# prashantpandeygit/solvingpapers

Measured on AMD Instinct MI355X. Metric: training tokens/sec, LLaMA3-8B-shape bf16, higher is better.
Workload: dtype bf16; 1 GPU; model=llama3_8b, global_batch=4, seq_len=8192, parallelism=dp1, micro_batch=1, grad_accum=4, params=8030261248

## Files before the change

### csrc/include/attn_common.h

```cpp
#pragma once
#include "spa_common.h"
#include <type_traits>

namespace spa {

template <int HD> constexpr int img_w() { return HD == 192 ? 256 : HD; }

typedef short s16x4 __attribute__((ext_vector_type(4)));
typedef int i32x4 __attribute__((ext_vector_type(4)));

constexpr float kRescaleThr = 8.f;

__device__ __forceinline__ f32x16 mfma32(const bf16x8& a, const bf16x8& b, const f32x16& c) {
  return __builtin_amdgcn_mfma_f32_32x32x16_bf16(a, b, c, 0, 0, 0);
}
__device__ __forceinline__ float fexp2(float x) { return __builtin_amdgcn_exp2f(x); }
__device__ __forceinline__ float halfmax(float x) {
  const auto r = __builtin_amdgcn_permlane32_swap(__float_as_uint(x), __float_as_uint(x), false, false);
  return fmaxf(__uint_as_float(r[0]), __uint_as_float(r[1]));
}
__device__ __forceinline__ float halfsum(float x) {
  const auto r = __builtin_amdgcn_permlane32_swap(__float_as_uint(x), __float_as_uint(x), false, false);
  return __uint_as_float(r[0]) + __uint_as_float(r[1]);
}
// ... 60 lines not shown
    for (int dt = 0; dt < NTR; ++dt) {
      const int c = 32 * dt + 16 * (g & 1) + 4 * pp;
      const int ch = c >> 3, within = c & 7;
      tra.v[dt] = ra * HD + 8 * (ch ^ swz<HD>(ra)) + within;
      trb.v[dt] = rb * HD + 8 * (ch ^ swz<HD>(rb)) + within;
    }
    SPA_DBG_LDS(row.v[NR - 1] + 7, 32 * HD);
    SPA_DBG_LDS(trb.v[NTR - 1] + 3, 16 * HD);
  }
};
__device__ __forceinline__ bf16x8 ld_row(const bf16* img, int off) {
  return *reinterpret_cast<const bf16x8*>(img + off);
}
__device__ __forceinline__ bf16x8 ld_tr(const bf16* img, int offa, int offb) {
  typedef __attribute__((address_space(3))) s16x4 lds_s4;
  const s16x4 a = __builtin_amdgcn_ds_read_tr16_b64_v4i16((lds_s4*)(img + offa));
  const s16x4 b = __builtin_amdgcn_ds_read_tr16_b64_v4i16((lds_s4*)(img + offb));
  const bf16x4 av = __builtin_bit_cast(bf16x4, a), bv = __builtin_bit_cast(bf16x4, b);
  return __builtin_shufflevector(av, bv, 0, 1, 2, 3, 4, 5, 6, 7);
}
template <int V> using IC = std::integral_constant<int, V>;

template <int N, int PER, int AHEAD, int PRE = 0>
__device__ __forceinline__ void chain_sched() {
  __builtin_amdgcn_sched_group_barrier(0x100, PRE + AHEAD * PER, 0);
#pragma unroll
  for (int i = 0; i < N - AHEAD; ++i) {
    __builtin_amdgcn_sched_group_barrier(0x008, 1, 0);
    __builtin_amdgcn_sched_group_barrier(0x100, PER, 0);
  }
  __builtin_amdgcn_sched_group_barrier(0x008, AHEAD, 0);
}

__device__ __forceinline__ unsigned lds_addr(const void* p) {
  return __builtin_amdgcn_readfirstlane((unsigned)(uintptr_t)p);
}
template <bool NT = false>
__device__ __forceinline__ void dma16_asm(__amdgpu_buffer_rsrc_t rs, unsigned voff, unsigned lds) {
  unsigned keep;
  if constexpr (NT)
    asm volatile("s_mov_b32 %0, m0\n\ts_mov_b32 m0, %3\n\ts_nop 0\n\tbuffer_load_dwordx4 %1, %2, 0 offen nt lds\n\ts_mov_b32 m0, %0"
                 : "=&s"(keep) : "v"(voff), "s"(rs), "s"(lds) : "memory");
  else
    asm volatile("s_mov_b32 %0, m0\n\ts_mov_b32 m0, %3\n\ts_nop 0\n\tbuffer_load_dwordx4 %1, %2, 0 offen lds\n\ts_mov_b32 m0, %0"
                 : "=&s"(keep) : "v"(voff), "s"(rs), "s"(lds) : "memory");
}

template <int HDC, int ROWS, int NT>
struct TileLoader {
  static constexpr int IW = img_w<HDC>();
  static constexpr int CPR = IW / 8;
  static constexpr int W = CPR < 16 ? CPR : 16;
  static constexpr int NC = CPR / W;
  static constexpr int R = NT / W;
  static constexpr int NP = ROWS / R;
  static constexpr int CH = NP * NC;
  static_assert(R % 16 == 0 && ROWS % R == 0 && NP >= 1, "tile/threads mismatch");
  bf16x8 r[CH];
  int voff;
  int loff;
  int ch;
  __device__ __forceinline__ void init(long stride, int tid) {
    const int rr = tid / W;
    ch = tid % W;
    voff = (int)(((long)rr * stride + ch * 8) * 2);
    loff = img_off<IW>(rr, ch);
  }
  __device__ __forceinline__ bool valid(int j) const { return HDC == IW || ch + 16 * j < HDC / 8; }
  __device__ __forceinline__ void load(const bf16* base, long stride, int row0, int nrows) {
#pragma unroll
    for (int ps = 0; ps < NP; ++ps) {
      const int r0 = row0 + ps * R;
      const int left = nrows - r0;
      const int bytes = left > 0 ? (int)(((long)(left - 1) * stride + HDC) * 2) : 0;
      const __amdgpu_buffer_rsrc_t rs =
          __builtin_amdgcn_make_buffer_rsrc((void*)(base + (long)r0 * stride), 0, bytes, 0x00020000);
#pragma unroll
      for (int j = 0; j < NC; ++j)
        if (valid(j))
          r[ps * NC + j] =
              __builtin_bit_cast(bf16x8, __builtin_amdgcn_raw_buffer_load_b128(rs, voff + 256 * j, 0, 0));
    }
  }
  __device__ __forceinline__ void store(bf16* img) const {
    SPA_DBG_LDS(loff + (NP - 1) * R * IW + 128 * (NC - 1) + 7, ROWS * IW);
#pragma unroll
    for (int ps = 0; ps < NP; ++ps)
#pragma unroll
      for (int j = 0; j < NC; ++j)
        if (valid(j)) *reinterpret_cast<bf16x8*>(img + loff + ps * R * IW + 128 * j) = r[ps * NC + j];
  }
};


}
```

### csrc/kernels/attention.hip

```cpp
#include "attn_common.h"
#include "attn_params.h"

SPA_DEBUG_TU("attention.hip")

namespace spa {



__device__ __forceinline__ unsigned mix32(unsigned x) {
  x ^= x >> 16; x *= 0x7feb352dU; x ^= x >> 15; x *= 0x846ca68bU; x ^= x >> 16;
  return x;
}
__device__ __forceinline__ unsigned drop_base(const AttnParams& p, int b, int h) {
  unsigned lo = p.seed_lo, hi = p.seed_hi;
  if (p.seed_ptr) {
    const uint64_t sd = (uint64_t)*p.seed_ptr;
    lo = (unsigned)(sd & 0xffffffffu);
    hi = (unsigned)(sd >> 32);
  }
  return mix32(lo ^ mix32(hi + (unsigned)(b * p.H + h) * 0x9E3779B9U));
}
__device__ __forceinline__ bool drop_keep(unsigned base, int q, int key, unsigned thr) {
  return (mix32(base + (unsigned)q * 0x85EBCA6BU + (unsigned)key * 0xC2B2AE35U) >> 8) >= thr;
}



__device__ __forceinline__ void q_block_map(const AttnParams& p, int nqb, bool causal, int& qb, int& b, int& h,
                                            int bi, int nblk) {
  const int G = p.H / p.Hkv;
  if (p.xcd) {
    const int cpx = nblk / 8;
    const int L = (bi % 8) * cpx + bi / 8;
    const int per_unit = nqb * G;
    const int u = L / per_unit, rem = L % per_unit;
    const int qr = rem / G, g = rem % G;
    qb = causal ? nqb - 1 - qr : qr;
    b = u / p.Hkv;
    h = (u % p.Hkv) * G + g;
  } else {
    const int nbh = p.H * p.B;
    const int bh = bi % nbh;
    qb = bi / nbh;
    if (causal) qb = nqb - 1 - qb;
    h = bh % p.H;
    b = bh / p.H;
  }
}

template <int HDK, int HDV> constexpr int attn_bn() { return (HDK >= 256 || HDV >= 256) ? 32 : 64; }

#ifndef FWD_PV_SCHED
#define FWD_PV_SCHED 1
#endif
template <int HDK, int HDV, int NW, bool CAUSAL, bool DROP>
__global__ __launch_bounds__(NW * 64) void attn_fwd_kernel(AttnParams p) {
  constexpr int BN = attn_bn<HDK, HDV>(), NSUB = BN / 32, BM = 32 * NW, KS = HDK / 16, DT = HDV / 32;
  constexpr int NT = NW * 64, IK = img_w<HDK>(), IV = img_w<HDV>();
  constexpr int TK = BN * IK, TV = BN * IV, TB = TK + TV;
  __shared__ __attribute__((aligned(16))) bf16 smem[2 * TB];
  const int tid = threadIdx.x, lane = tid & 63, wave = tid >> 6;
  const int lq = lane & 31, hh = lane >> 5;
  const int nqb = cdiv(p.Tq, BM);
  const int si = blockIdx.x % p.ksplit;
  int qb, b, h;
  q_block_map(p, nqb, CAUSAL, qb, b, h, blockIdx.x / p.ksplit, gridDim.x / p.ksplit);
  const int hk = h / (p.H / p.Hkv);
  SPA_DBG_CHECK(qb, nqb);
  SPA_DBG_CHECK(hk, p.Hkv);
  (void)SPA_DBG_BRH(b, 0, 1, h, p.H);
  const int q0 = __builtin_amdgcn_readfirstlane(qb * BM + wave * 32);
  const int q = q0 + lq;
  const float c = p.scale_log2;
  const int vcol = blockIdx.y * p.vhalf;
  unsigned dbase = 0;
  if constexpr (DROP) dbase = drop_base(p, b, h);

  bf16x8 qf[KS];
  {
    const bf16* qp = p.q + b * p.sqb + (long)q * p.sqt + h * p.sqh + 8 * hh;
#pragma unroll
    for (int s = 0; s < KS; ++s) qf[s] = q < p.Tq ? *reinterpret_cast<const bf16x8*>(qp + 16 * s) : zero8();
  }
  f32x16 o[DT];
#pragma unroll
  for (int i = 0; i < DT; ++i) o[i] = splat16(0.f);
  float m = -1e30f, l = 0.f;

  int kend = p.Tk;
  if (CAUSAL) kend = min(p.Tk, qb * BM + BM + p.causal_off);
  const int wave_kend = q0 >= p.Tq ? 0 : CAUSAL ? min(p.Tk, q0 + 32 + p.causal_off) : p.Tk;
  const int ntiles_all = kend > 0 ? cdiv(kend, BN) : 0;
  const int kper = cdiv(ntiles_all, p.ksplit);
  const int jbeg = min(ntiles_all, si * kper);
  const int ntiles = min(ntiles_all, jbeg + kper) - jbeg;
  const int kb0 = jbeg * BN;

  const bf16* kbase = p.k + b * p.skb + hk * p.skh;
  const bf16* vbase = p.v + b * p.svb + hk * p.svh + vcol;
  TileLoader<HDK, BN, NT> lk;
  TileLoader<HDV, BN, NT> lv;
  lk.init(p.skt, tid);
  lv.init(p.svt, tid);
  if (ntiles > 0) {
    lk.load(kbase, p.skt, kb0, p.Tk);
    lv.load(vbase, p.svt, kb0, p.Tk);
    lk.store(smem);
    lv.store(smem + TK);
    if (ntiles > 1) { lk.load(kbase, p.skt, kb0 + BN, p.Tk); lv.load(vbase, p.svt, kb0 + BN, p.Tk); }
  }
  __syncthreads();
  LdsOff<IK> offk;
  LdsOff<IV> offv;
  offk.init(lane);
  offv.init(lane);
  auto mask = [&](f32x16& s, const int k0) {
#pragma unroll
    for (int r = 0; r < 16; ++r) {
      const int key = k0 + (r & 3) + 8 * (r >> 2) + 4 * hh;
      if (key >= p.Tk || (CAUSAL && key > q + p.causal_off)) s[r] = -INFINITY;
    }
  };
  auto softmax = [&](f32x16& s) {
    float mx = s[0];
#pragma unroll
    for (int r = 1; r < 16; ++r) mx = fmaxf(mx, s[r]);
    const float mxs = halfmax(mx) * c;
    if (mxs > m + kRescaleThr) {
      const float alpha = fexp2(m - mxs);
      l *= alpha;
#pragma unroll
      for (int i = 0; i < DT; ++i)
#pragma unroll
        for (int r = 0; r < 16; ++r) o[i][r] *= alpha;
      m = mxs;
    }
    const float nm = -m;
    float ls = 0.f;
#pragma unroll
    for (int r = 0; r < 16; ++r) {
      const float e = fexp2(fmaf(s[r], c, nm));
      s[r] = e;
      ls += e;
    }
    l += ls;
  };
  auto dropout = [&](f32x16& s, const int k0) {
#pragma unroll
    for (int r = 0; r < 16; ++r) {
      const int key = k0 + (r & 3) + 8 * (r >> 2) + 4 * hh;
      s[r] = drop_keep(dbase, q, key, p.drop_thr) ? s[r] * p.drop_scale : 0.f;
    }
  };
  auto body = [&](const int j, auto bufc) {
    constexpr int BUF = decltype(bufc)::value;
    const int k0 = kb0 + j * BN;
    const bf16* Ks = smem + BUF * TB;
    const bf16* Vs = Ks + TK;
    if (j + 1 < ntiles) {
      bf16* Kn = smem + (1 - BUF) * TB;
      lk.store(Kn);
      lv.store(Kn + TK);
      if (j + 2 < ntiles) { lk.load(kbase, p.skt, k0 + 2 * BN, p.Tk); lv.load(vbase, p.svt, k0 + 2 * BN, p.Tk); }
    }
#pragma unroll
    for (int t = 0; t < NSUB; ++t) {
      const int ks0 = k0 + 32 * t;
      if (ks0 < wave_kend) {
        bf16x8 kr[KS];
#pragma unroll
        for (int ks = 0; ks < KS; ++ks) kr[ks] = ld_row(Ks + 32 * t * IK, offk.row[ks]);
        f32x16 s = mfma32(kr[0], qf[0], splat16(0.f));
#pragma unroll
        for (int ks = 1; ks < KS; ++ks) s = mfma32(kr[ks], qf[ks], s);
        __builtin_amdgcn_sched_group_barrier(0x100, KS, 0);
        __builtin_amdgcn_sched_group_barrier(0x008, KS, 0);
        const bool need_mask = (ks0 + 32 > p.Tk) || (CAUSAL && ks0 + 31 > q0 + p.causal_off);
        if (need_mask) mask(s, ks0);
        softmax(s);
        if constexpr (DROP) dropout(s, ks0);
        const bf16x8 pa = pack_acc(s, 0), pb = pack_acc(s, 1);
#pragma unroll
        for (int dt = 0; dt < DT; ++dt) {
          o[dt] = mfma32(ld_tr(Vs + 32 * t * IV, offv.tra[dt], offv.trb[dt]), pa, o[dt]);
          o[dt] = mfma32(ld_tr(Vs + (32 * t + 16) * IV, offv.tra[dt], offv.trb[dt]), pb, o[dt]);
        }
        if (FWD_PV_SCHED) chain_sched<2 * DT, 2, 3>();
      }
    }
    __syncthreads();
  };
#pragma unroll
  for (int s = 0; s < KS; ++s) asm volatile("" ::"v"(qf[s]));
  for (int j = 0; j < ntiles; j += 2) {
    body(j, IC<0>{});
    if (j + 1 < ntiles) body(j + 1, IC<1>{});
  }
  l = halfsum(l);
  if (p.ksplit > 1) {
    if (q < p.Tq && SPA_DBG_OK(si, p.ksplit)) {
      const long row = (((long)si * p.B + b) * p.H + h) * p.Tq + q;
      SPA_DBG_CHECK(row, (long)p.ksplit * p.B * p.H * p.Tq);
      float* dst = p.part + row * p.part_ld + vcol;
#pragma unroll
      for (int dt = 0; dt < DT; ++dt)
#pragma unroll
        for (int g = 0; g < 4; ++g) {
          f32x4 w;
#pragma unroll
          for (int i = 0; i < 4; ++i) w[i] = o[dt][4 * g + i];
          *reinterpret_cast<f32x4*>(dst + 32 * dt + 8 * g + 4 * hh) = w;
        }
      if (hh == 0 && blockIdx.y == 0) {
        float2 ml;
        ml.x = m;
        ml.y = l;
        reinterpret_cast<float2*>(p.mlpart)[row] = ml;
      }
    }
    return;
  }
  const float inv = l > 0.f ? 1.f / l : 0.f;
  if (q < p.Tq && SPA_DBG_BRH(b, q, p.Tq, h, p.H)) {
    bf16* op = p.out + b * p.sob + (long)q * p.sot + h * p.soh + vcol;
#pragma unroll
    for (int dt = 0; dt < DT; ++dt)
#pragma unroll
      for (int g = 0; g < 4; ++g) {
        bf16x4 w;
#pragma unroll
        for (int i = 0; i < 4; ++i) w[i] = (bf16)(o[dt][4 * g + i] * inv);
        *reinterpret_cast<bf16x4*>(op + 32 * dt + 8 * g + 4 * hh) = w;
      }
    if (hh == 0 && p.lse)
      p.lse[((long)b * p.H + h) * p.Tq + q] = (l > 0.f) ? (m + __log2f(l)) * 0.69314718055994531f : INFINITY;
  }
}

template <bool CAUSAL>
__global__ __launch_bounds__(512) void attn_fwd256p_kernel(AttnParams p) {
  constexpr int HD = 256, BN = 32, BM = 128, KS = HD / 16, DH = 4, NT = 512;
  constexpr int TI = BN * HD;
  constexpr int PS = 4 * 2 * 64 * 8;
  __shared__ __attribute__((aligned(16))) bf16 smem[4 * TI + 2 * PS];
  __shared__ __attribute__((aligned(16))) float arow[2][4][64];
  const int tid = threadIdx.x, lane = tid & 63;
  const int wave = __builtin_amdgcn_readfirstlane(tid >> 6);
  const int grp = wave & 3, role = wave >> 2;
  const int lq = lane & 31, hh = lane >> 5;
  const int nqb = cdiv(p.Tq, BM);
  const int si = blockIdx.x % p.ksplit;
  int qb, b, h;
  q_block_map(p, nqb, CAUSAL, qb, b, h, blockIdx.x / p.ksplit, gridDim.x / p.ksplit);
  const int hk = h / (p.H / p.Hkv);
  SPA_DBG_CHECK(qb, nqb);
  SPA_DBG_CHECK(hk, p.Hkv);
  (void)SPA_DBG_BRH(b, 0, 1, h, p.H);
  const int q0 = __builtin_amdgcn_readfirstlane(qb * BM + grp * 32);
  const int q = q0 + lq;
  const float c = p.scale_log2;

  int kend = p.Tk;
  if (CAUSAL) kend = min(p.Tk, qb * BM + BM + p.causal_off);
  const int wave_kend = q0 >= p.Tq ? 0 : CAUSAL ? min(p.Tk, q0 + 32 + p.causal_off) : p.Tk;
  const int ntiles_all = kend > 0 ? cdiv(kend, BN) : 0;
  const int kper = cdiv(ntiles_all, p.ksplit);
  const int jbeg = min(ntiles_all, si * kper);
  const int ntiles = min(ntiles_all, jbeg + kper) - jbeg;
  const int kb0 = jbeg * BN;

  const bf16* kbase = p.k + b * p.skb + hk * p.skh;
  const bf16* vbase = p.v + b * p.svb + hk * p.svh;
  TileLoader<HD, BN, NT> lk, lv;
  lk.init(p.skt, tid);
  lv.init(p.svt, tid);
  if (ntiles > 0) {
    lk.load(kbase, p.skt, kb0, p.Tk);
    lk.store(smem);
    lv.load(vbase, p.svt, kb0, p.Tk);
// ... 858 lines not shown
        }
        const bf16x8 sa = pack_acc(ds, 0), sb = pack_acc(ds, 1);
        if constexpr (DSOUT) {
          const int qt = qtp + t, kt = kw0 >> 5;
          if ((!CAUSAL || kt <= qt) && qt < p.ds_nqt && kt < p.ds_nkt) {
            const __amdgpu_buffer_rsrc_t dsr = __builtin_amdgcn_make_buffer_rsrc(
                (void*)(p.dsbuf + ((long)b * p.Hkv + hk) * p.ds_kvstride), 0, (int)(p.ds_kvstride * 2), 0x00020000);
            const int bo = (int)(ds_index(qt, kt, hp - hk * (p.H / p.Hkv), p.H / p.Hkv, p.ds_nkt, CAUSAL) * 2048);
            SPA_DBG_CHECK(bo / 2048, p.ds_kvstride / 1024);
            const int vo = 16 * ds_slot(0, (int)(__lane_id() >> 5), (int)(__lane_id() & 31));
            __builtin_amdgcn_raw_buffer_store_b128(__builtin_bit_cast(i32x4, sa), dsr, vo, bo, 0);
            __builtin_amdgcn_raw_buffer_store_b128(__builtin_bit_cast(i32x4, sb), dsr, vo + 128, bo, 0);
          }
          __builtin_amdgcn_sched_barrier(0);
        }
        DK3_TICK(1);
        if constexpr (DVS) {
#pragma unroll
          for (int dt = 0; dt < DTX; ++dt) {
            acc[dt] = mfma32(ld_tr(Dpr + 32 * t * IWV, offv.tra[DTX + dt], offv.trb[DTX + dt]), pa, acc[dt]);
            acc[dt] = mfma32(ld_tr(Dpr + (32 * t + 16) * IWV, offv.tra[DTX + dt], offv.trb[DTX + dt]), pb, acc[dt]);
          }
          if (DKDV3_DVS_SCHED) chain_sched<2 * DTX, 2, 2>();
        } else {
#pragma unroll
          for (int dt = 0; dt < DTK; ++dt) {
            acc[dt] = mfma32(ld_tr(Qp + 32 * t * IWK, offk.tra[dt], offk.trb[dt]), sa, acc[dt]);
            acc[dt] = mfma32(ld_tr(Qp + (32 * t + 16) * IWK, offk.tra[dt], offk.trb[dt]), sb, acc[dt]);
          }
          if (DKDV3_SCHED) chain_sched<2 * DTK, 2, 2, 2>();
        }
        __builtin_amdgcn_sched_barrier(0);
        DK3_TICK(2);
      }
    }
    prev_act = cur;
    __syncthreads();
    DK3_TICK(3);
  };
#pragma unroll
  for (int s = 0; s < KSX; ++s) asm volatile("" ::"v"(xf[s]));
  if (role == 0) {
    for (int k = 0; k <= total; k += 3) {
      interval(k, IC<0>{}, IC<0>{});
      if (k + 1 <= total) interval(k + 1, IC<1>{}, IC<0>{});
      if (k + 2 <= total) interval(k + 2, IC<2>{}, IC<0>{});
    }
  } else {
    for (int k = 0; k <= total; k += 3) {
      interval(k, IC<0>{}, IC<1>{});
      if (k + 1 <= total) interval(k + 1, IC<1>{}, IC<1>{});
      if (k + 2 <= total) interval(k + 2, IC<2>{}, IC<1>{});
    }
  }
  if constexpr (DVS) {
    store_kv_grad<HDV>(p, acc, false, b, hk, key, split, hh, role * DTX);
  } else if constexpr (HDK == HDV) {
    store_kv_grad<HDK>(p, acc, role == 1, b, hk, key, split, hh);
  } else {
    if (role == 1) {
      f32x16 ak[DTK];
#pragma unroll
      for (int i = 0; i < DTK; ++i) ak[i] = acc[i];
      store_kv_grad<HDK>(p, ak, true, b, hk, key, split, hh);
    } else {
      f32x16 av[DTV];
#pragma unroll
      for (int i = 0; i < DTV; ++i) av[i] = acc[i];
      store_kv_grad<HDV>(p, av, false, b, hk, key, split, hh);
    }
  }
#if SPA_DKDV3_STAMP
  DK3_TICK(4);
  if (p.stamp != nullptr && lane < 8) {
    long long v = 0;
#pragma unroll
    for (int i = 0; i < 5; ++i) v = lane == i ? seg[i] : v;
    v = lane == 5 ? (long long)(total + 1) : lane == 6 ? ts_ - t_start : v;
    p.stamp[((long)blockIdx.x * 8 + wave) * 8 + lane] = v;
  }
#endif
}

template <int HD, bool CAUSAL, bool NT>
__global__ __launch_bounds__(256, 2) void attn_bwd_dq_ds_kernel(AttnParams p) {
  static_assert(HD == 128, "dq_ds: head dim 128 (K tile = 4 KiB-row images of 256 B)");
  constexpr int DT = HD / 32, KIMG = 32 * HD, WSLOT = 2 * 1024, SLOT = KIMG + 4 * WSLOT, NSLOT = 3;
  __shared__ __attribute__((aligned(16))) bf16 smem[NSLOT * SLOT];
  const int tid = threadIdx.x, lane = tid & 63;
  const int wave = __builtin_amdgcn_readfirstlane(tid >> 6);
  const int hh = lane >> 5;
  const int G = p.H / p.Hkv;
  const int nq64 = cdiv(p.Tq, 64);
  const int upkv = nq64 * G;
  const int wgpkv = cdiv(upkv, 4);
  const int nbkv = p.B * p.Hkv;
  const int bkv = blockIdx.x % nbkv;
  const int w = CAUSAL ? wgpkv - 1 - (int)(blockIdx.x / nbkv) : (int)(blockIdx.x / nbkv);
  const int b = bkv / p.Hkv, hk = bkv % p.Hkv;
  SPA_DBG_CHECK(b, p.B);
  const int u = 4 * w + wave;
  const bool uvalid = u < upkv;
  const int qb = uvalid ? u / G : 0;
  const int h = hk * G + (uvalid ? u % G : 0);
  auto unit_steps = [&](int uu) {
    const int qbb = uu / G;
    return CAUSAL ? cdiv(min(p.Tk, qbb * 64 + 64 + p.causal_off), 32) : cdiv(p.Tk, 32);
  };
  const int nsteps_w = uvalid ? unit_steps(u) : 0;
  const int nsteps = unit_steps(min(4 * w + 3, upkv - 1));

  const bf16* kbase = p.k + b * p.skb + hk * p.skh;
  unsigned kvo[2];
#pragma unroll
  for (int j = 0; j < 2; ++j) {
    const int r = 8 * wave + 4 * j + (lane >> 4);
    kvo[j] = (unsigned)(((long)r * p.skt + 8 * ((lane & 15) ^ swz<HD>(r))) * 2);
  }
  const bf16* dskv = p.dsbuf + ((long)b * p.Hkv + hk) * p.ds_kvstride;
  const int g = h - hk * G;
  auto live = [&](int qt, int kt) { return uvalid && qt < p.ds_nqt && (!CAUSAL || kt <= qt); };
  auto issue = [&](int j, int slot) {
    bf16* sl = smem + slot * SLOT;
    const int key0 = 32 * j;
    const long kbytes = key0 < p.Tk ? ((long)(p.Tk - key0 - 1) * p.skt + HD) * 2 : 0;
    const __amdgpu_buffer_rsrc_t rk = __builtin_amdgcn_make_buffer_rsrc(
        (void*)(kbase + (long)key0 * p.skt), 0, (int)min(kbytes, 0x7fffffffL), 0x00020000);
#pragma unroll
    for (int jj = 0; jj < 2; ++jj) dma16_asm(rk, kvo[jj], lds_addr(sl + (8 * wave + 4 * jj) * HD));
    const bool lv = live(2 * qb + 1, j) || live(2 * qb, j);
    if (lv) SPA_DBG_CHECK(ds_index(2 * qb, j, g, G, p.ds_nkt, CAUSAL), p.ds_kvstride / 1024);
    const bf16* src = lv ? dskv + ds_index(2 * qb, j, g, G, p.ds_nkt, CAUSAL) * 1024 : p.dsbuf;
    const __amdgpu_buffer_rsrc_t rd = __builtin_amdgcn_make_buffer_rsrc((void*)src, 0, lv ? 4096 : 0, 0x00020000);
    bf16* dst = sl + KIMG + wave * WSLOT;
#pragma unroll
    for (int jj = 0; jj < 4; ++jj) dma16_asm<NT>(rd, (unsigned)(lane * 16 + jj * 1024), lds_addr(dst + jj * 512));
  };
  LdsOff<HD> off;
  off.init(lane);
  int dso[2];
  {
    const int g = (lane >> 4) & 1, i = lane & 15, q = i >> 2, pp = i & 3;
#pragma unroll
    for (int ab = 0; ab < 2; ++ab) {
      const int key = 4 * hh + q + 8 * ab;
      dso[ab] = 8 * ds_slot(g, pp & 1, key) + 4 * (pp >> 1);
    }
  }
  f32x16 acc[2][DT];
#pragma unroll
  for (int t = 0; t < 2; ++t)
#pragma unroll
    for (int i = 0; i < DT; ++i) acc[t][i] = splat16(0.f);

  auto compute = [&](int j, const bf16* sl) {
    if (j >= nsteps_w) return;
    const bf16* Ks = sl;
    const bf16* Dw = sl + KIMG + wave * WSLOT;
    const bool l0 = live(2 * qb, j), l1 = live(2 * qb + 1, j);
#pragma unroll
    for (int s = 0; s < 2; ++s) {
      bf16x8 kt[DT];
#pragma unroll
      for (int dt = 0; dt < DT; ++dt) kt[dt] = ld_tr(Ks + 16 * s * HD, off.tra[dt], off.trb[dt]);
      const bf16x8 d0 = ld_tr(Dw + 512 * s, dso[0], dso[1]);
      const bf16x8 d1 = ld_tr(Dw + 1024 + 512 * s, dso[0], dso[1]);
      if (l0) {
#pragma unroll
        for (int dt = 0; dt < DT; ++dt) acc[0][dt] = mfma32(kt[dt], d0, acc[0][dt]);
      }
      if (l1) {
#pragma unroll
        for (int dt = 0; dt < DT; ++dt) acc[1][dt] = mfma32(kt[dt], d1, acc[1][dt]);
      }
    }
  };
  if (nsteps > 0) issue(0, 0);
  if (nsteps > 1) issue(1, 1);
  for (int j = 0; j < nsteps; j += 3) {
#pragma unroll
    for (int r = 0; r < 3; ++r) {
      const int jj = j + r;
      if (jj < nsteps) {
        if (jj + 1 < nsteps) asm volatile("s_waitcnt vmcnt(6)" ::: "memory");
        else asm volatile("s_waitcnt vmcnt(0)" ::: "memory");
        asm volatile("s_waitcnt lgkmcnt(0)" ::: "memory");
        __builtin_amdgcn_s_barrier();
        if (jj + 2 < nsteps) issue(jj + 2, (r + 2) % 3);
        compute(jj, smem + r * SLOT);
      }
    }
  }
  if (!uvalid) return;
#pragma unroll
  for (int t = 0; t < 2; ++t) {
    const int q = qb * 64 + 32 * t + (lane & 31);
    if (q >= p.Tq || !SPA_DBG_BRH(b, q, p.Tq, h, p.H)) continue;
    bf16* op = p.dq + b * p.sdqb + (long)q * p.sdqt + h * p.sdqh;
#pragma unroll
    for (int dt = 0; dt < DT; ++dt)
#pragma unroll
      for (int g = 0; g < 4; ++g) {
        bf16x4 wv;
#pragma unroll
        for (int i = 0; i < 4; ++i) wv[i] = (bf16)(acc[t][dt][4 * g + i] * p.scale);
        *reinterpret_cast<bf16x4*>(op + 32 * dt + 8 * g + 4 * hh) = wv;
      }
  }
}

template <int HDK, bool CAUSAL, bool NT>
__global__ __launch_bounds__(256, 2) void attn_bwd_dq_ds256_kernel(AttnParams p) {
  static_assert(HDK == 256 || HDK == 192, "dq_ds256: q/k head dim 192 or 256");
  constexpr int HD = 256, DT = HDK / 32, KIMG = 32 * HD, WSLOT = 1024, SLOT = KIMG + 4 * WSLOT, NSLOT = 3;
  __shared__ __attribute__((aligned(16))) bf16 smem[NSLOT * SLOT];
  const int tid = threadIdx.x, lane = tid & 63;
  const int wave = __builtin_amdgcn_readfirstlane(tid >> 6);
  const int hh = lane >> 5;
  const int G = p.H / p.Hkv;
  const int nqt = cdiv(p.Tq, 32);
  const int upkv = nqt * G;
  const int wgpkv = cdiv(upkv, 4);
  const int nbkv = p.B * p.Hkv;
  const int bkv = blockIdx.x % nbkv;
  const int w = CAUSAL ? wgpkv - 1 - (int)(blockIdx.x / nbkv) : (int)(blockIdx.x / nbkv);
  const int b = bkv / p.Hkv, hk = bkv % p.Hkv;
  SPA_DBG_CHECK(b, p.B);
  const int u = 4 * w + wave;
  const bool uvalid = u < upkv;
  const int qt = uvalid ? u / G : 0;
  const int h = hk * G + (uvalid ? u % G : 0);
  auto unit_steps = [&](int uu) {
    const int qtt = uu / G;
    return CAUSAL ? cdiv(min(p.Tk, qtt * 32 + 32 + p.causal_off), 32) : cdiv(p.Tk, 32);
  };
  const int nsteps_w = uvalid ? unit_steps(u) : 0;
  const int nsteps = unit_steps(min(4 * w + 3, upkv - 1));

  const bf16* kbase = p.k + b * p.skb + hk * p.skh;
  unsigned kvo[4];
#pragma unroll
  for (int j = 0; j < 4; ++j) {
    const int r = 8 * wave + 2 * j + (lane >> 5);
    kvo[j] = (unsigned)(((long)r * p.skt + 8 * ((lane & 31) ^ swz<HD>(r))) * 2);
  }
  const bf16* dskv = p.dsbuf + ((long)b * p.Hkv + hk) * p.ds_kvstride;
  const int g = h - hk * G;
  auto live = [&](int kt) { return uvalid && qt < p.ds_nqt && (!CAUSAL || kt <= qt); };
  auto issue = [&](int j, int slot) {
    bf16* sl = smem + slot * SLOT;
    const int key0 = 32 * j;
    const long kbytes = key0 < p.Tk ? ((long)(p.Tk - key0 - 1) * p.skt + HDK) * 2 : 0;
    const __amdgpu_buffer_rsrc_t rk = __builtin_amdgcn_make_buffer_rsrc(
        (void*)(kbase + (long)key0 * p.skt), 0, (int)min(kbytes, 0x7fffffffL), 0x00020000);
#pragma unroll
    for (int jj = 0; jj < 4; ++jj) dma16_asm(rk, kvo[jj], lds_addr(sl + (8 * wave + 2 * jj) * HD));
    const bool lv = live(j);
    if (lv) SPA_DBG_CHECK(ds_index(qt, j, g, G, p.ds_nkt, CAUSAL), p.ds_kvstride / 1024);
    const bf16* src = lv ? dskv + ds_index(qt, j, g, G, p.ds_nkt, CAUSAL) * 1024 : p.dsbuf;
    const __amdgpu_buffer_rsrc_t rd = __builtin_amdgcn_make_buffer_rsrc((void*)src, 0, lv ? 2048 : 0, 0x00020000);
    bf16* dst = sl + KIMG + wave * WSLOT;
#pragma unroll
// ... 178 lines not shown
template <int HD>
__global__ __launch_bounds__(256) void attn_delta_kernel(AttnParams p) {
  constexpr int TPR = HD / 8, RPB = 256 / TPR;
  const long row = (long)blockIdx.x * RPB + threadIdx.x / TPR;
  const int t = threadIdx.x % TPR;
  const long nrows = (long)p.B * p.Tq * p.H;
  float acc = 0.f;
  long b = 0, q = 0, h = 0;
  if (row < nrows) {
    h = row % p.H;
    q = (row / p.H) % p.Tq;
    b = row / ((long)p.H * p.Tq);
    float a[8], c[8];
    load8(p.dout + b * p.sdob + q * p.sdot + h * p.sdoh + 8 * t, a);
    load8(p.o + b * p.sob + q * p.sot + h * p.soh + 8 * t, c);
#pragma unroll
    for (int i = 0; i < 8; ++i) acc += a[i] * c[i];
  }
#pragma unroll
  for (int o = TPR / 2; o > 0; o >>= 1) acc += __shfl_xor(acc, o, TPR);
  if (row < nrows && t == 0 && SPA_DBG_BRH(b, q, p.Tq, h, p.H)) p.delta[(b * p.H + h) * p.Tq + q] = acc;
}
template <int HD>
__global__ __launch_bounds__(256) void attn_dq_store_kernel(AttnParams p) {
  constexpr int TPR = HD / 8;
  const long n = (long)p.B * p.Tq * p.H * TPR;
  for (long i = blockIdx.x * 256L + threadIdx.x; i < n; i += (long)gridDim.x * 256) {
    const int t = i % TPR;
    const long row = i / TPR;
    const long h = row % p.H, q = (row / p.H) % p.Tq, b = row / ((long)p.H * p.Tq);
    float a[8];
    load8(p.dqacc + row * HD + 8 * t, a);
#pragma unroll
    for (int k = 0; k < 8; ++k) a[k] *= p.scale;
    if (SPA_DBG_BRH(b, q, p.Tq, h, p.H)) store8(p.dq + b * p.sdqb + q * p.sdqt + h * p.sdqh + 8 * t, a);
  }
}


static void check_qkv(const at::Tensor& t, const char* n) {
  TORCH_CHECK(t.is_cuda() && t.scalar_type() == at::kBFloat16, n, " must be a bf16 HIP tensor");
  TORCH_CHECK(t.dim() == 4, n, " must be [B, T, H, hd]");
  TORCH_CHECK(t.stride(3) == 1, n, " must be contiguous in hd");
  TORCH_CHECK(((uintptr_t)t.data_ptr() % 16) == 0 && t.stride(1) % 8 == 0 && t.stride(2) % 8 == 0 &&
                  t.stride(0) % 8 == 0,
              n, ": rows must be 16-byte aligned");
}

template <int HDK, int HDV> constexpr int fwd_waves() {
  return (HDK <= 192 && HDV <= 192) || (HDK == 256 && HDV == 128) ? 8 : 4;
}
template <int HDK, int HDV> constexpr int dq_waves() { return (HDK <= 128 && HDV <= 128) ? 8 : 4; }

#define HDKV_SWITCH(HK, HV, ...)                                                                   \
  if (HK == 64 && HV == 64) { constexpr int HDK_ = 64, HDV_ = 64; __VA_ARGS__; }                  \
  else if (HK == 128 && HV == 128) { constexpr int HDK_ = 128, HDV_ = 128; __VA_ARGS__; }         \
  else if (HK == 256 && HV == 256) { constexpr int HDK_ = 256, HDV_ = 256; __VA_ARGS__; }         \
  else if (HK == 192 && HV == 128) { constexpr int HDK_ = 192, HDV_ = 128; __VA_ARGS__; }         \
  else TORCH_CHECK(false, "flash attention: (qk, v) head dims must be (64,64), (128,128), (256,256) or (192,128)");

static void fill_strides(AttnParams& p, const at::Tensor& q, const at::Tensor& k, const at::Tensor& v) {
  p.sqb = q.stride(0); p.sqt = q.stride(1); p.sqh = q.stride(2);
  p.skb = k.stride(0); p.skt = k.stride(1); p.skh = k.stride(2);
  p.svb = v.stride(0); p.svt = v.stride(1); p.svh = v.stride(2);
}

static int xcd_order(int B, int Hkv) {
  const char* e = getenv("SPA_ATTN_XCD");
  if (e && atoi(e) == 0) return 0;
  return ((long)B * Hkv) % 8 == 0 ? 1 : 0;
}

static void fill_dropout(AttnParams& p, double dropout_p, int64_t seed, const c10::optional<at::Tensor>& seed_t) {
  if (seed_t) {
    TORCH_CHECK(seed_t->is_cuda() && seed_t->scalar_type() == at::kLong && seed_t->numel() >= 1,
                "attention seed_t: int64 device tensor");
    p.seed_ptr = seed_t->data_ptr<int64_t>();
  }
  TORCH_CHECK(dropout_p >= 0.0 && dropout_p < 1.0, "attention dropout p must be in [0, 1)");
  p.seed_lo = (unsigned)(seed & 0xffffffffu);
  p.seed_hi = (unsigned)(((uint64_t)seed >> 32) & 0xffffffffu);
  p.drop_thr = (unsigned)std::llround(dropout_p * 16777216.0);
  p.drop_scale = (float)(1.0 / (1.0 - dropout_p));
}

static int attn_ksplit(long blocks, int ntk) {
  const char* e = getenv("SPA_ATTN_KSPLIT");
  if (e) return std::max(1, std::min(atoi(e), std::max(1, ntk)));
  int ks = 1;
  while (blocks * ks < 512 && ks < 8 && ntk / (2 * ks) >= 4) ks *= 2;
  return ks;
}

std::vector<at::Tensor> attn_fwd(const at::Tensor& q, const at::Tensor& k, const at::Tensor& v, double scale,
                                 bool causal, double dropout_p, int64_t seed,
                                 const c10::optional<at::Tensor>& seed_t) {
  check_qkv(q, "q"); check_qkv(k, "k"); check_qkv(v, "v");
  const int B = q.size(0), Tq = q.size(1), H = q.size(2), HDK = q.size(3), HDV = v.size(3);
  const int Tk = k.size(1), Hkv = k.size(2);
  TORCH_CHECK(k.size(0) == B && v.size(0) == B && v.size(1) == Tk && v.size(2) == Hkv && k.size(3) == HDK,
              "attn: shape mismatch");
  TORCH_CHECK(H % Hkv == 0, "attn: H must be a multiple of Hkv");
  const bool drop = dropout_p > 0.0;
  TORCH_CHECK(!drop || HDK == HDV, "attn: dropout needs equal q/k and v head dims");
  DeviceGuard g(q.device());
  auto out = at::empty({B, Tq, H, HDV}, q.options());
  auto lse = at::empty({B, H, Tq}, q.options().dtype(at::kFloat));
  AttnParams p{};
  p.q = (const bf16*)q.data_ptr(); p.k = (const bf16*)k.data_ptr(); p.v = (const bf16*)v.data_ptr();
  p.out = (bf16*)out.data_ptr(); p.lse = lse.data_ptr<float>();
  p.B = B; p.H = H; p.Hkv = Hkv; p.Tq = Tq; p.Tk = Tk;
  fill_strides(p, q, k, v);
  fill_dropout(p, dropout_p, seed, seed_t);
  p.sob = out.stride(0); p.sot = out.stride(1); p.soh = out.stride(2);
  p.scale = (float)scale; p.scale_log2 = (float)(scale * 1.4426950408889634);
  p.causal_off = Tk - Tq;
  p.hsplit = 1;
  p.ksplit = 1;
  p.xcd = xcd_order(B, Hkv);
  if (B * Tq * H == 0) return {out, lse};
  auto st = stream();
  const char* f2e = getenv("SPA_ATTN_FWD256");
  const bool pshare = !(f2e && atoi(f2e) == 0) && HDK == 256 && HDV == 256 && !drop;
  const char* sve = getenv("SPA_ATTN_SPLITV");
  const bool splitv = !pshare && !(sve && atoi(sve) == 0) && HDK == 256 && HDV == 256 && !drop;
  const int nw = splitv || pshare ? 8 : (HDK <= 192 && HDV <= 192) || (HDK == 256 && HDV == 128) ? 8 : 4;
  const int blocks = cdiv(Tq, pshare ? 128 : 32 * nw) * H * B * (splitv ? 2 : 1);
  const int ntk = cdiv(Tk, (HDK >= 256 || HDV >= 256) ? 32 : 64);
  p.ksplit = attn_ksplit(blocks, ntk);
  at::Tensor part;
  if (p.ksplit > 1) {
    const long rows = (long)B * H * Tq;
    part = at::empty({(long)p.ksplit * rows * (HDV + 2)}, q.options().dtype(at::kFloat));
    p.part = part.data_ptr<float>();
    p.part_ld = HDV;
    p.mlpart = p.part + (long)p.ksplit * rows * HDV;
  }
  const int gx = blocks / (splitv ? 2 : 1) * p.ksplit;
  if (pshare) {
    if (causal) attn_fwd256p_kernel<true><<<gx, 512, 0, st>>>(p);
    else attn_fwd256p_kernel<false><<<gx, 512, 0, st>>>(p);
  } else if (splitv) {
    p.vhalf = 128;
    if (causal) attn_fwd_kernel<256, 128, 8, true, false><<<dim3(gx, 2), 512, 0, st>>>(p);
    else attn_fwd_kernel<256, 128, 8, false, false><<<dim3(gx, 2), 512, 0, st>>>(p);
  } else {
    HDKV_SWITCH(HDK, HDV, {
      constexpr int NW = fwd_waves<HDK_, HDV_>();
      constexpr bool SQ = HDK_ == HDV_;
      if (drop) {
        if constexpr (SQ) {
          if (causal) attn_fwd_kernel<HDK_, HDV_, NW, true, true><<<gx, NW * 64, 0, st>>>(p);
          else attn_fwd_kernel<HDK_, HDV_, NW, false, true><<<gx, NW * 64, 0, st>>>(p);
        }
      } else {
        if (causal) attn_fwd_kernel<HDK_, HDV_, NW, true, false><<<gx, NW * 64, 0, st>>>(p);
        else attn_fwd_kernel<HDK_, HDV_, NW, false, false><<<gx, NW * 64, 0, st>>>(p);
      }
    });
  }
  if (p.ksplit > 1) {
    const long n = (long)B * H * Tq * (HDV / 8);
    HDKV_SWITCH(HDK, HDV, { attn_fwd_merge_kernel<HDV_><<<(int)cdiv(n, 256L), 256, 0, st>>>(p); });
  }
  SPA_LAUNCH_CHECK();
  return {out, lse};
}

template <int HDK, int HDV, bool DROP>
static void launch_bwd(AttnParams& p, bool causal, bool fused, int dkdv_mode, int nkv, hipStream_t st,
                       const at::TensorOptions& bf16_opts) {
  constexpr int NW = dq_waves<HDK, HDV>();
  constexpr int MT = (HDK <= 128 && HDV <= 128) ? 2 : 1;
  constexpr bool PAIRED_OK = HDK == HDV && HDK <= 128 && !DROP;
  const int g2 = nkv * p.hsplit;
  if constexpr (HDK == HDV && HDK <= 128 && !DROP) {
    if (fused) {
      const long rows = (long)p.B * p.Tq * p.H;
      attn_delta_kernel<HDK><<<(int)cdiv(rows, 256 / (HDK / 8)), 256, 0, st>>>(p);
      if (causal) attn_bwd_dkdv_kernel<HDK, HDV, true, MT, true, false><<<g2, 256, 0, st>>>(p);
      else attn_bwd_dkdv_kernel<HDK, HDV, false, MT, true, false><<<g2, 256, 0, st>>>(p);
      const long n = rows * (HDK / 8);
      attn_dq_store_kernel<HDK><<<(int)std::min<long>((n + 255) / 256, 65536), 256, 0, st>>>(p);
      return;
    }
  }
  if constexpr (HDK == 128 && HDV == 128 && !DROP) {
    const char* de = getenv("SPA_ATTN_DQ_DS");
    const bool want = !(de && atoi(de) == 0);
    const long kv_bytes = 2 * ds_kv_elems(cdiv(p.Tq, 64), cdiv(p.Tk, 32), p.H / p.Hkv, causal);
    if (want && p.hsplit == 1 && p.Tk > 0 && dkdv_mode == 0 && (!causal || p.causal_off == 0) &&
        kv_bytes < 0x7fffffffL) {
      const long rows = (long)p.B * p.Tq * p.H;
      const char* v5e = getenv("SPA_ATTN_DKDV5");
      const bool v5 = !(v5e && atoi(v5e) == 0);
      if (!v5) attn_delta_kernel<HDK><<<(int)cdiv(rows, 256 / (HDK / 8)), 256, 0, st>>>(p);
      p.ds_nqt = cdiv(p.Tq, 32);
      p.ds_nkt = cdiv(p.Tk, 32);
      p.ds_kvstride = ds_kv_elems(cdiv(p.Tq, 64), p.ds_nkt, p.H / p.Hkv, causal);
      at::Tensor dsb = at::empty({(long)p.B * p.Hkv * p.ds_kvstride}, bf16_opts);
      p.dsbuf = (bf16*)dsb.data_ptr();
      at::Tensor rowk;
      if (v5) {
        p.rowk_ld = cdiv(p.Tq, 64) * 64;
        rowk = at::empty({(long)p.B * p.H * 2 * p.rowk_ld}, bf16_opts.dtype(at::kFloat));
        p.rowk = rowk.data_ptr<float>();
        launch_dkdv5(p, causal, st);
      } else if (causal) attn_bwd_dkdv3_kernel<HDK, HDV, true, true><<<nkv, 512, 0, st>>>(p);
      else attn_bwd_dkdv3_kernel<HDK, HDV, false, true><<<nkv, 512, 0, st>>>(p);
      const int G = p.H / p.Hkv;
      const int wg = cdiv(cdiv(p.Tq, 64) * G, 4) * p.B * p.Hkv;
      const char* ne = getenv("SPA_ATTN_DS_NT");
      const bool nt = !(ne && atoi(ne) == 0);
      if (nt) {
        if (causal) attn_bwd_dq_ds_kernel<HDK, true, true><<<wg, 256, 0, st>>>(p);
        else attn_bwd_dq_ds_kernel<HDK, false, true><<<wg, 256, 0, st>>>(p);
      } else {
        if (causal) attn_bwd_dq_ds_kernel<HDK, true, false><<<wg, 256, 0, st>>>(p);
        else attn_bwd_dq_ds_kernel<HDK, false, false><<<wg, 256, 0, st>>>(p);
      }
      return;
    }
  }
  if constexpr (((HDK == 256 && HDV == 256) || (HDK == 192 && HDV == 128)) && !DROP) {
    const char* de = getenv("SPA_ATTN_DQ_DS");
    const int dsm = de ? atoi(de) : 1;
    const bool want = dsm != 0;
    const int G = p.H / p.Hkv;
    const long kv_bytes = 2 * ds_kv_elems(cdiv(p.Tq, 64), cdiv(p.Tk, 32), G, causal);
    const int wg = cdiv(cdiv(p.Tq, 32) * G, 4) * p.B * p.Hkv;
    if (want && (wg >= 512 || dsm == 2) && p.Tk > 0 && dkdv_mode == 0 && (!causal || p.causal_off == 0) &&
        kv_bytes < 0x7fffffffL) {
      const long rows = (long)p.B * p.Tq * p.H;
      attn_delta_kernel<HDV><<<(int)cdiv(rows, 256 / (HDV / 8)), 256, 0, st>>>(p);
      p.ds_nqt = cdiv(p.Tq, 32);
      p.ds_nkt = cdiv(p.Tk, 32);
      p.ds_kvstride = ds_kv_elems(cdiv(p.Tq, 64), p.ds_nkt, G, causal);
      at::Tensor dsb = at::empty({(long)p.B * p.Hkv * p.ds_kvstride}, bf16_opts);
      p.dsbuf = (bf16*)dsb.data_ptr();
      const int g2 = nkv * p.hsplit;
      bool paired_mla = false, dvs = false;
      AttnParams pk = p;
      at::Tensor dkpart;
      if constexpr (HDK == 256 && HDV == 256) {
        const char* ve = getenv("SPA_ATTN_DKDV256");
        dvs = !(ve && atoi(ve) == 0) && G % p.hsplit == 0;
        if (dvs) {
          if (causal) attn_bwd_dkdv3_kernel<HDK, HDV, true, true, true><<<g2, 512, 0, st>>>(p);
          else attn_bwd_dkdv3_kernel<HDK, HDV, false, true, true><<<g2, 512, 0, st>>>(p);
          int hs2 = p.hsplit;
          while (nkv * hs2 < 1024 && hs2 < G) {
            int d = hs2 + 1;
            while (G % d) ++d;
            hs2 = d;
          }
          pk.hsplit = hs2;
          if (hs2 > 1) {
            dkpart = at::empty({(long)hs2 * p.B * p.Tk * p.Hkv * HDK}, bf16_opts.dtype(at::kFloat));
            pk.dkacc = dkpart.data_ptr<float>();
          }
          if (causal) attn_bwd_dk_ds256_kernel<true, true><<<nkv * hs2, 256, 0, st>>>(pk);
          else attn_bwd_dk_ds256_kernel<false, true><<<nkv * hs2, 256, 0, st>>>(pk);
        }
      }
      if constexpr (HDK == 192 && HDV == 128) {
        const char* me = getenv("SPA_ATTN_DKDV_MLA");
        paired_mla = p.hsplit == 1 && !(me && atoi(me) == 1);
        if (paired_mla) {
          if (causal) attn_bwd_dkdv3_kernel<HDK, HDV, true, true><<<g2, 512, 0, st>>>(p);
          else attn_bwd_dkdv3_kernel<HDK, HDV, false, true><<<g2, 512, 0, st>>>(p);
        }
      }
      if (!paired_mla && !dvs) {
        if (causal) attn_bwd_dkdv_kernel<HDK, HDV, true, 1, false, false, true><<<g2, 256, 0, st>>>(p);
        else attn_bwd_dkdv_kernel<HDK, HDV, false, 1, false, false, true><<<g2, 256, 0, st>>>(p);
      }
      const char* ne = getenv("SPA_ATTN_DS_NT");
      const bool nt = !(ne && atoi(ne) == 0);
      if (nt) {
        if (causal) attn_bwd_dq_ds256_kernel<HDK, true, true><<<wg, 256, 0, st>>>(p);
        else attn_bwd_dq_ds256_kernel<HDK, false, true><<<wg, 256, 0, st>>>(p);
      } else {
        if (causal) attn_bwd_dq_ds256_kernel<HDK, true, false><<<wg, 256, 0, st>>>(p);
        else attn_bwd_dq_ds256_kernel<HDK, false, false><<<wg, 256, 0, st>>>(p);
      }
      const long kr = (long)p.B * p.Tk * p.Hkv;
      if ((dvs ? pk : p).hsplit > 1)
        attn_kv_reduce_kernel<HDK><<<(int)std::min<long>((kr * (HDK / 8) + 255) / 256, 65536), 256, 0, st>>>(dvs ? pk : p, 1);
      if (p.hsplit > 1)
        attn_kv_reduce_kernel<HDV><<<(int)std::min<long>((kr * (HDV / 8) + 255) / 256, 65536), 256, 0, st>>>(p, 0);
      return;
    }
  }
  const int grid = cdiv(p.Tq, 32 * NW) * p.H * p.B;
  p.ksplit = p.Tk > 0 ? attn_ksplit(grid, cdiv(p.Tk, attn_bn<HDK, HDV>())) : 1;
  at::Tensor dqpart;
  if (p.ksplit > 1) {
    dqpart = at::empty({(long)p.ksplit * p.B * p.Tq * p.H * HDK}, bf16_opts.dtype(at::kFloat));
    p.part = dqpart.data_ptr<float>();
    p.part_ld = HDK;
  }
  if (causal) attn_bwd_dq_kernel<HDK, HDV, NW, true, DROP><<<grid * p.ksplit, NW * 64, 0, st>>>(p);
  else attn_bwd_dq_kernel<HDK, HDV, NW, false, DROP><<<grid * p.ksplit, NW * 64, 0, st>>>(p);
// ... 132 lines not shown
```

Measured before the change: 22450 tokens/s.

## Add fast-path interior tile loops to attention fwd and dq backward kernels

Splits the forward attention K-loop and the backward dq_ds loop into a fast interior phase, where tiles are known to be full and unmasked, and a general tail. The fast phase drops per-tile bounds checks, causal masking and wave_kend tests. It also advances K/V and ds pointers incrementally with full-tile buffer descriptors instead of rebuilding descriptors with computed byte limits. This cuts scalar bookkeeping and branch overhead in the hot loops, at the cost of more code paths and reliance on the correctness of the fast-range computation. The path is enabled by default and can be turned off with SPA_ATTN_BOOK=0.

```diff
diff --git a/csrc/include/attn_common.h b/csrc/include/attn_common.h
--- a/csrc/include/attn_common.h
+++ b/csrc/include/attn_common.h
@@ -166,6 +166,16 @@
               __builtin_bit_cast(bf16x8, __builtin_amdgcn_raw_buffer_load_b128(rs, voff + 256 * j, 0, 0));
     }
   }
+  __device__ __forceinline__ void load_full(const bf16* tile, int bytes, int rstep) {
+    const __amdgpu_buffer_rsrc_t rs = __builtin_amdgcn_make_buffer_rsrc((void*)tile, 0, bytes, 0x00020000);
+#pragma unroll
+    for (int ps = 0; ps < NP; ++ps)
+#pragma unroll
+      for (int j = 0; j < NC; ++j)
+        if (valid(j))
+          r[ps * NC + j] =
+              __builtin_bit_cast(bf16x8, __builtin_amdgcn_raw_buffer_load_b128(rs, voff + 256 * j, ps * rstep, 0));
+  }
   __device__ __forceinline__ void store(bf16* img) const {
     SPA_DBG_LDS(loff + (NP - 1) * R * IW + 128 * (NC - 1) + 7, ROWS * IW);
 #pragma unroll
diff --git a/csrc/kernels/attention.hip b/csrc/kernels/attention.hip
--- a/csrc/kernels/attention.hip
+++ b/csrc/kernels/attention.hip
@@ -53,7 +53,7 @@
 #ifndef FWD_PV_SCHED
 #define FWD_PV_SCHED 1
 #endif
-template <int HDK, int HDV, int NW, bool CAUSAL, bool DROP>
+template <int HDK, int HDV, int NW, bool CAUSAL, bool DROP, bool BOOK = false>
 __global__ __launch_bounds__(NW * 64) void attn_fwd_kernel(AttnParams p) {
   constexpr int BN = attn_bn<HDK, HDV>(), NSUB = BN / 32, BM = 32 * NW, KS = HDK / 16, DT = HDV / 32;
   constexpr int NT = NW * 64, IK = img_w<HDK>(), IV = img_w<HDV>();
@@ -152,12 +152,28 @@
       s[r] = drop_keep(dbase, q, key, p.drop_thr) ? s[r] * p.drop_scale : 0.f;
     }
   };
-  auto body = [&](const int j, auto bufc) {
+  const bf16* kn = kbase;
+  const bf16* vn = vbase;
+  const long kstep = BN * p.skt, vstep = BN * p.svt;
+  const int kfull = (int)(((BN - 1) * p.skt + HDK) * 2), vfull = (int)(((BN - 1) * p.svt + HDV) * 2);
+  const int krow = (int)(TileLoader<HDK, BN, NT>::R * p.skt * 2), vrow = (int)(TileLoader<HDV, BN, NT>::R * p.svt * 2);
+  auto body = [&](const int j, auto bufc, auto fastc) {
     constexpr int BUF = decltype(bufc)::value;
+    constexpr bool FAST = decltype(fastc)::value;
     const int k0 = kb0 + j * BN;
     const bf16* Ks = smem + BUF * TB;
     const bf16* Vs = Ks + TK;
-    if (j + 1 < ntiles) {
+    if constexpr (FAST) {
+      bf16* Kn = smem + (1 - BUF) * TB;
+      lk.store(Kn);
+      lv.store(Kn + TK);
+      SPA_DBG_ASSERT(kn - kbase == (long)(k0 + 2 * BN) * p.skt && k0 + 3 * BN <= p.Tk, kn - kbase, j);
+      SPA_DBG_ASSERT(vn - vbase == (long)(k0 + 2 * BN) * p.svt && j + 2 < ntiles, vn - vbase, j);
+      lk.load_full(kn, kfull, krow);
+      lv.load_full(vn, vfull, vrow);
+      kn += kstep;
+      vn += vstep;
+    } else if (j + 1 < ntiles) {
       bf16* Kn = smem + (1 - BUF) * TB;
       lk.store(Kn);
       lv.store(Kn + TK);
@@ -166,7 +182,7 @@
 #pragma unroll
     for (int t = 0; t < NSUB; ++t) {
       const int ks0 = k0 + 32 * t;
-      if (ks0 < wave_kend) {
+      if (FAST || ks0 < wave_kend) {
         bf16x8 kr[KS];
 #pragma unroll
         for (int ks = 0; ks < KS; ++ks) kr[ks] = ld_row(Ks + 32 * t * IK, offk.row[ks]);
@@ -175,8 +191,12 @@
         for (int ks = 1; ks < KS; ++ks) s = mfma32(kr[ks], qf[ks], s);
         __builtin_amdgcn_sched_group_barrier(0x100, KS, 0);
         __builtin_amdgcn_sched_group_barrier(0x008, KS, 0);
-        const bool need_mask = (ks0 + 32 > p.Tk) || (CAUSAL && ks0 + 31 > q0 + p.causal_off);
-        if (need_mask) mask(s, ks0);
+        if constexpr (FAST) {
+          SPA_DBG_ASSERT(ks0 + 32 <= p.Tk && ks0 < wave_kend && !(CAUSAL && ks0 + 31 > q0 + p.causal_off), ks0, q0);
+        } else {
+          const bool need_mask = (ks0 + 32 > p.Tk) || (CAUSAL && ks0 + 31 > q0 + p.causal_off);
+          if (need_mask) mask(s, ks0);
+        }
         softmax(s);
         if constexpr (DROP) dropout(s, ks0);
         const bf16x8 pa = pack_acc(s, 0), pb = pack_acc(s, 1);
@@ -192,9 +212,22 @@
   };
 #pragma unroll
   for (int s = 0; s < KS; ++s) asm volatile("" ::"v"(qf[s]));
-  for (int j = 0; j < ntiles; j += 2) {
-    body(j, IC<0>{});
-    if (j + 1 < ntiles) body(j + 1, IC<1>{});
+  int j = 0;
+  if constexpr (BOOK) {
+    const int nfull = (p.Tk - kb0) / BN;
+    const int nvis = !CAUSAL ? nfull : q0 + p.causal_off + 1 > kb0 ? (q0 + p.causal_off + 1 - kb0) / BN : 0;
+    const int jm = q0 >= p.Tq ? -1 : min(min(ntiles, nfull) - 4, nvis - 2);
+    const int jfast = __builtin_amdgcn_readfirstlane(jm >= 0 ? (jm / 2) * 2 + 2 : 0);
+    kn = kbase + (long)(kb0 + 2 * BN) * p.skt;
+    vn = vbase + (long)(kb0 + 2 * BN) * p.svt;
+    for (; j < jfast; j += 2) {
+      body(j, IC<0>{}, std::true_type{});
+      body(j + 1, IC<1>{}, std::true_type{});
+    }
+  }
+  for (; j < ntiles; j += 2) {
+    body(j, IC<0>{}, std::false_type{});
+    if (j + 1 < ntiles) body(j + 1, IC<1>{}, std::false_type{});
   }
   l = halfsum(l);
   if (p.ksplit > 1) {
@@ -1219,7 +1252,7 @@
 #endif
 }
 
-template <int HD, bool CAUSAL, bool NT>
+template <int HD, bool CAUSAL, bool NT, bool BOOK = true>
 __global__ __launch_bounds__(256, 2) void attn_bwd_dq_ds_kernel(AttnParams p) {
   static_assert(HD == 128, "dq_ds: head dim 128 (K tile = 4 KiB-row images of 256 B)");
   constexpr int DT = HD / 32, KIMG = 32 * HD, WSLOT = 2 * 1024, SLOT = KIMG + 4 * WSLOT, NSLOT = 3;
@@ -1314,7 +1347,64 @@
   };
   if (nsteps > 0) issue(0, 0);
   if (nsteps > 1) issue(1, 1);
-  for (int j = 0; j < nsteps; j += 3) {
+  int j = 0;
+  if constexpr (BOOK) {
+    const int e0 = !uvalid ? 0 : CAUSAL ? 2 * qb + 1 : nsteps;
+    const int e1 = !(uvalid && 2 * qb + 1 < p.ds_nqt) ? 0 : CAUSAL ? 2 * qb + 2 : nsteps;
+    const int nboth = min(min(e0, e1), nsteps_w);
+    const int nissue = min(min(max(e0, e1), nsteps), p.Tk / 32);
+    const int lim = min(nboth - 2, nissue - 4);
+    const int jfast = __builtin_amdgcn_readfirstlane(lim > 0 ? 3 * cdiv(lim, 3) : 0);
+    if (jfast > 0) {
+      const long kstep = 32 * p.skt;
+      const int dstep = 2 * G * 1024;
+      const int kfull = (int)((31 * p.skt + HD) * 2);
+      const bf16* kp = kbase + 2 * kstep;
+      const bf16* dp = dskv + ds_index(2 * qb, 2, g, G, p.ds_nkt, CAUSAL) * 1024;
+      __amdgpu_buffer_rsrc_t rk = __builtin_amdgcn_make_buffer_rsrc((void*)kp, 0, kfull, 0x00020000);
+      __amdgpu_buffer_rsrc_t rd = __builtin_amdgcn_make_buffer_rsrc((void*)dp, 0, 4096, 0x00020000);
+      for (; j < jfast; j += 3) {
+#pragma unroll
+        for (int r = 0; r < 3; ++r) {
+#if SPA_DEBUG_BOUNDS
+          SPA_DBG_CHECK((dp - dskv) / 1024, p.ds_kvstride / 1024);
+          SPA_DBG_ASSERT(dp - dskv == ds_index(2 * qb, j + r + 2, g, G, p.ds_nkt, CAUSAL) * 1024, dp - dskv, j + r + 2);
+          SPA_DBG_ASSERT(kp - kbase == (long)(32 * (j + r + 2)) * p.skt && 32 * (j + r + 2) + 32 <= p.Tk, kp - kbase,
+                         j + r + 2);
+#endif
+          asm volatile("" ::"s"(rk), "s"(rd));
+          asm volatile("s_waitcnt vmcnt(6)" ::: "memory");
+          asm volatile("s_waitcnt lgkmcnt(0)" ::: "memory");
+          __builtin_amdgcn_s_barrier();
+          bf16* sl = smem + ((r + 2) % 3) * SLOT;
+#pragma unroll
+          for (int jj = 0; jj < 2; ++jj) dma16_asm(rk, kvo[jj], lds_addr(sl + (8 * wave + 4 * jj) * HD));
+          bf16* dst = sl + KIMG + wave * WSLOT;
+#pragma unroll
+          for (int jj = 0; jj < 4; ++jj) dma16_asm<NT>(rd, (unsigned)(lane * 16 + jj * 1024), lds_addr(dst + jj * 512));
+          kp += kstep;
+          dp += dstep;
+          rk = __builtin_amdgcn_make_buffer_rsrc((void*)kp, 0, kfull, 0x00020000);
+          rd = __builtin_amdgcn_make_buffer_rsrc((void*)dp, 0, 4096, 0x00020000);
+          const bf16* Ks = smem + r * SLOT;
+          const bf16* Dw = Ks + KIMG + wave * WSLOT;
+#pragma unroll
+          for (int s = 0; s < 2; ++s) {
+            bf16x8 kt[DT];
+#pragma unroll
+            for (int dt = 0; dt < DT; ++dt) kt[dt] = ld_tr(Ks + 16 * s * HD, off.tra[dt], off.trb[dt]);
+            const bf16x8 d0 = ld_tr(Dw + 512 * s, dso[0], dso[1]);
+            const bf16x8 d1 = ld_tr(Dw + 1024 + 512 * s, dso[0], dso[1]);
+#pragma unroll
+            for (int dt = 0; dt < DT; ++dt) acc[0][dt] = mfma32(kt[dt], d0, acc[0][dt]);
+#pragma unroll
+            for (int dt = 0; dt < DT; ++dt) acc[1][dt] = mfma32(kt[dt], d1, acc[1][dt]);
+          }
+        }
+      }
+    }
+  }
+  for (; j < nsteps; j += 3) {
 #pragma unroll
     for (int r = 0; r < 3; ++r) {
       const int jj = j + r;
@@ -1659,6 +1749,11 @@
   p.seed_hi = (unsigned)(((uint64_t)seed >> 32) & 0xffffffffu);
   p.drop_thr = (unsigned)std::llround(dropout_p * 16777216.0);
   p.drop_scale = (float)(1.0 / (1.0 - dropout_p));
+}
+
+static bool attn_book() {
+  const char* e = getenv("SPA_ATTN_BOOK");
+  return !(e && atoi(e) == 0);
 }
 
 static int attn_ksplit(long blocks, int ntk) {
@@ -1730,6 +1825,9 @@
           if (causal) attn_fwd_kernel<HDK_, HDV_, NW, true, true><<<gx, NW * 64, 0, st>>>(p);
           else attn_fwd_kernel<HDK_, HDV_, NW, false, true><<<gx, NW * 64, 0, st>>>(p);
         }
+      } else if (HDK_ == 128 && HDV_ == 128 && attn_book()) {
+        if (causal) attn_fwd_kernel<HDK_, HDV_, NW, true, false, HDK_ == 128 && HDV_ == 128><<<gx, NW * 64, 0, st>>>(p);
+        else attn_fwd_kernel<HDK_, HDV_, NW, false, false, HDK_ == 128 && HDV_ == 128><<<gx, NW * 64, 0, st>>>(p);
       } else {
         if (causal) attn_fwd_kernel<HDK_, HDV_, NW, true, false><<<gx, NW * 64, 0, st>>>(p);
         else attn_fwd_kernel<HDK_, HDV_, NW, false, false><<<gx, NW * 64, 0, st>>>(p);
@@ -1789,13 +1887,18 @@
       const int wg = cdiv(cdiv(p.Tq, 64) * G, 4) * p.B * p.Hkv;
       const char* ne = getenv("SPA_ATTN_DS_NT");
       const bool nt = !(ne && atoi(ne) == 0);
-      if (nt) {
-        if (causal) attn_bwd_dq_ds_kernel<HDK, true, true><<<wg, 256, 0, st>>>(p);
-        else attn_bwd_dq_ds_kernel<HDK, false, true><<<wg, 256, 0, st>>>(p);
-      } else {
-        if (causal) attn_bwd_dq_ds_kernel<HDK, true, false><<<wg, 256, 0, st>>>(p);
-        else attn_bwd_dq_ds_kernel<HDK, false, false><<<wg, 256, 0, st>>>(p);
-      }
+      auto launch_dq = [&](auto bookc) {
+        constexpr bool BOOK = decltype(bookc)::value;
+        if (nt) {
+          if (causal) attn_bwd_dq_ds_kernel<HDK, true, true, BOOK><<<wg, 256, 0, st>>>(p);
+          else attn_bwd_dq_ds_kernel<HDK, false, true, BOOK><<<wg, 256, 0, st>>>(p);
+        } else {
+          if (causal) attn_bwd_dq_ds_kernel<HDK, true, false, BOOK><<<wg, 256, 0, st>>>(p);
+          else attn_bwd_dq_ds_kernel<HDK, false, false, BOOK><<<wg, 256, 0, st>>>(p);
+        }
+      };
+      if (attn_book()) launch_dq(std::true_type{});
+      else launch_dq(std::false_type{});
       return;
     }
   }
```

Result: no change. 22550 tokens/s (median of 6 runs) (+0.4%).
